# HyperBitGore/deflate.hpp

Measured on AMD Instinct MI355X. Metric: GB/s deflate+inflate on 1 GiB buffer at 1/2/4/8 MI355X; ratio vs reference, higher is better.
Workload: dtype u8; 1 GPU; deflate level 2 + inflate round trip of a per-GPU 1 GiB 'repeat' corpus (SURVEY App. B), device-resident; corpus=repeat, bytes_per_gpu=1073741824, level=2, segment_bytes=32768, parallelism=shard1

## Files before the change

### deflate.hpp_amd/csrc/deflate_kernels.hip

```cpp
#include "dmx_device.h"
#include "dmx_internal.h"
#include "huff_fit.h"

namespace dmx {

constexpr int DF_NT = 1024;
constexpr int DF_CHUNK = 258;
constexpr int df_hash_bits(int seg) {
    return seg >= 32768 ? 12 : 11;
}
constexpr int DF_L3_DEPTH = 16;
constexpr uint32_t DF_L3_LONG = 16;
constexpr uint32_t DF_L3_RP = 512;
constexpr bool df_early(int seg) { return seg >= 32768; }
constexpr uint32_t EM_ALL_LITERALS = 0xFFFFFFFFu;


__device__ __forceinline__ int df_tid() {
    int t = threadIdx.x;
    asm volatile("" : "+v"(t));
    return t;
}

__device__ uint32_t block_excl_scan(uint32_t v, uint32_t* scratch, uint32_t* total) {
// ... 158 lines not shown
    while (L < maxl) {
        const uint32_t o = L + 16 * sub;
        const uint32_t ip = (p + o) >> 2, sp = (p + o) & 3, iq = (q + o) >> 2, sq = (q + o) & 3;
        uint32_t a[5], b[5];
#pragma unroll
        for (int k = 0; k < 5; k++) {
            a[k] = w[ip + k];
            b[k] = w[iq + k];
        }
        uint32_t x = 0, off = 0;
#pragma unroll
        for (int k = 0; k < 4; k++) {
            const uint32_t d = __builtin_amdgcn_alignbyte(a[k + 1], a[k], sp) ^
                               __builtin_amdgcn_alignbyte(b[k + 1], b[k], sq);
            if (!x && d) {
                x = d;
                off = 4 * k;
            }
        }
        uint32_t v = x ? 16 * sub + off + ((uint32_t)__builtin_ctz(x) >> 3) : 64u;
        v = min(v, xor_lane<1>(v));
        v = min(v, xor_lane<2>(v));
        if (v < 64) {
            L += v;
            break;
        }
        L += 64;
    }
    return min(L, maxl);
}

__device__ __forceinline__ uint8_t data_byte(const uint32_t* w, uint32_t p) {
    return (uint8_t)(w[p >> 2] >> ((p & 3) * 8));
}

__device__ __forceinline__ uint32_t fixed_lit_len(uint32_t s) {
    return s < 144 ? 8 : s < 256 ? 9 : s < 280 ? 7 : 8;
}
__device__ __forceinline__ uint32_t fixed_lit_code(uint32_t s) {
    uint32_t c = s < 144 ? 0x30 + s : s < 256 ? 0x190 + (s - 144) : s < 280 ? s - 256 : 0xC0 + (s - 280);
    return bitrev(c, fixed_lit_len(s));
}


template <int SEG, bool EARLY>
struct DfBufs;
template <int SEG>
struct DfBufs<SEG, false> {
    uint32_t data32[SEG / 4 + 32];
    alignas(16) uint16_t cand[SEG + 8];
    alignas(16) uint32_t U[2 << df_hash_bits(SEG)];
};
template <int SEG>
struct DfBufs<SEG, true> {
    static constexpr int BW = SEG / 4 + 32;
    static_assert((2 << df_hash_bits(SEG)) * 4 == SEG, "the table fills an image buffer's SEG bytes");
    alignas(16) uint32_t buf[2][BW];
    alignas(16) uint16_t cand[SEG + 8];
};
template <int SEG>
struct DfSmem : DfBufs<SEG, df_early(SEG)> {
    static constexpr bool EARLY = df_early(SEG);
    static constexpr int NWALK = (SEG + DF_CHUNK - 1) / DF_CHUNK;
    static constexpr int HB = df_hash_bits(SEG);
    static constexpr int HT = 1 << HB;
    static constexpr int UW = 2 * HT;
// ... 122 lines not shown
    uint32_t head = (16u - (off & 15u)) & 15u;
    if (((reinterpret_cast<uintptr_t>(src) + head) & 15) != 0 || head > n) head = n;
    for (uint32_t i = t; i < head; i += DF_NT) dbytes[off + i] = src[i];
    const uint32_t nvec = (n - head) / 16;
    const uint4* s4 = reinterpret_cast<const uint4*>(src + head);
    uint4* d4 = reinterpret_cast<uint4*>(dbytes + off + head);
    for (uint32_t i = t; i < nvec; i += DF_NT) d4[i] = s4[i];
    for (uint32_t i = head + 16 * nvec + t; i < n; i += DF_NT) dbytes[off + i] = src[i];
}

template <int SEG, bool L3, bool BATCH, bool DICT, bool PIPE = false>
__device__ __forceinline__ void deflate_segment(const DeflateArgs& A, DfSmem<SEG>& S, uint64_t seg,
                                                uint32_t& staged, [[maybe_unused]] uint32_t iw) {
    constexpr bool EARLY = DfSmem<SEG>::EARLY;
    uint32_t *data32, *U;
    if constexpr (EARLY) {
        data32 = &S.buf[0][0] + iw;
        U = &S.buf[0][0] + ((uint32_t)DfSmem<SEG>::BW - iw);
    } else {
        data32 = S.data32;
        U = S.U;
    }
    [[maybe_unused]] constexpr int NWALK = DfSmem<SEG>::NWALK;
    constexpr int HT = DfSmem<SEG>::HT;
    constexpr int NMAP = SEG / 32;
    const int t = df_tid();
    const DfSegAddr sa = df_seg_addr<SEG, BATCH, DICT>(A, seg);
    const uint32_t D = DICT ? sa.dlen : 0u;
    const uint32_t nb = D + sa.nb;
    constexpr int level = L3 ? 3 : 2;
    uint8_t* const dbytes = reinterpret_cast<uint8_t*>(data32);
    constexpr bool TERMRUN = !L3 && SEG >= 32768;
    constexpr uint32_t RUN_NONE = 0xFFFFFFFFu;
    DMX_PHASE(A.dbg, seg, 0);

    {
        const uint8_t* src = sa.src;
        const uint32_t nvec = nb / 16;
        if (staged) {
        } else if (DICT && D) {
            df_load_at(dbytes, 0, sa.dict, D, t);
            df_load_at(dbytes, D, src, nb - D, t);
        } else if ((((uintptr_t)src) & 15) == 0) {
            const uint4* s4 = reinterpret_cast<const uint4*>(src);
            uint4* d4 = reinterpret_cast<uint4*>(data32);
            for (uint32_t i = t; i < nvec; i += DF_NT) d4[i] = s4[i];
            for (uint32_t i = nvec * 16 + t; i < nb; i += DF_NT) dbytes[i] = src[i];
        } else {
            for (uint32_t i = t; i < nb; i += DF_NT) dbytes[i] = src[i];
        }
        for (uint32_t i = nb + t; i < ((nb + 3) & ~3u) + 32; i += DF_NT) dbytes[i] = 0;
        if (t < NMAP) S.tokmap[t] = 0;
        if (t == 0) S.sh[46] = 0;
        if (TERMRUN && t == 1) S.sh[45] = RUN_NONE;
        if (TERMRUN && t == 2) S.sh[43] = 0;
        if (t >= 48 && t < 63) S.sh[t] = 0;
        if (level >= 2 && EARLY) {
            uint4* const u4 = reinterpret_cast<uint4*>(U);
            for (int i = t; i < 2 * HT / 4; i += DF_NT) u4[i] = make_uint4(0, 0, 0, 0);
        } else if (level >= 2)
            for (int i = t; i < 2 * HT; i += DF_NT) U[i] = 0;
    }
    if constexpr (EARLY) df_lds_barrier();
    else __syncthreads();
    DMX_PHASE(A.dbg, seg, 1);
    staged = 0;

    if (level != 0) {
        [[maybe_unused]] uint32_t run_lo = RUN_NONE, run_d = 0;
        [[maybe_unused]] uint32_t run_e = RUN_NONE;
        [[maybe_unused]] float run_rcp = 0.f;
        if (level >= 2) {
            constexpr uint32_t HB = DfSmem<SEG>::HB;
            const uint2* const tab = reinterpret_cast<const uint2*>(U);
            uint32_t* const cand32 = reinterpret_cast<uint32_t*>(S.cand);
            constexpr uint32_t NOH = 0xFFFFFFFFu;
            struct RoundState {
                uint32_t h0, h1, p0, f0, f1;
                bool ok0, ok1;
            };
            bool skipped = false;
            auto run_rounds = [&](auto rpc) {
                constexpr uint32_t RP = decltype(rpc)::value;
                constexpr uint32_t NR = SEG / RP;
                constexpr uint32_t TAGB = NR <= 16 ? 4 : NR <= 32 ? 5 : NR <= 64 ? 6 : 7;
                static_assert(NR <= 128, "round number is at most 7 bits");
                constexpr uint32_t FPB = 17 - TAGB;
                const bool act = RP >= 2 * DF_NT || t < (int)(RP / 2);
                const uint32_t tt = RP >= 2 * DF_NT ? (uint32_t)t : (uint32_t)t & (RP / 2 - 1);
                constexpr bool SKIP = RP == 2 * DF_NT;
                uint32_t skip_d = 0, skip_end = 0, wait = 0, backoff = 1;
                skipped = false;
                bool pend = false;
                auto round = [&](uint32_t r0, uint32_t rr, RoundState& cur, const RoundState& prev, auto full) {
                    constexpr bool FULL = decltype(full)::value;
                    const uint32_t p0 = r0 + 2 * tt, p1 = p0 + 1;
                    if (SKIP && skip_d) {
                        if (r0 + RP <= skip_end || (!TERMRUN && skip_end >= nb)) {
                            if (FULL || p0 < nb)
                                cand32[p0 >> 1] = (FULL || p0 + 4 <= nb ? skip_d : 0u) |
                                                  ((FULL || p1 + 4 <= nb ? skip_d : 0u) << 16);
                            cur = RoundState{NOH, NOH, p0, 0, 0, false, false};
                            skipped = true;
                            return;
                        }
                        skip_d = 0;
                    }
                    uint32_t dlr = 0;
                    if (SKIP && pend) dlr = S.sh[44];
                    const uint32_t i0 = p0 >> 2, sh = p0 & 3;
                    const uint32_t wa = data32[i0], wb = data32[i0 + 1];
                    const uint32_t k0 = __builtin_amdgcn_alignbyte(wb, wa, sh);
                    const uint32_t k1 = __builtin_amdgcn_alignbyte(wb, wa, sh + 1);
                    const uint32_t prod0 = k0 * 0x1E35A7BDu;
                    const uint32_t prod1 = k1 * 0x1E35A7BDu;
                    const bool ok0 = act && (FULL || p0 + 4 <= nb), ok1 = act && (FULL || p1 + 4 <= nb);
                    const uint32_t h0 = ok0 ? prod0 >> (32 - HB) : NOH, h1 = ok1 ? prod1 >> (32 - HB) : NOH;
                    const uint32_t fa0 = (prod0 >> (32 - HB - 16)) & 0xFFFFu, fa1 = (prod1 >> (32 - HB - 16)) & 0xFFFFu;
                    const uint32_t hl = (uint32_t)__builtin_amdgcn_update_dpp((int)NOH, (int)h1, 0x111, 0xF, 0xF, false);
                    const uint32_t rtag = rr << (32 - TAGB);
                    if (ok0 && h0 != hl)
                        atomicMax(&U[2 * h0 + 1], rtag | ((0x7FFFu - p0) << FPB) | (fa0 >> (16 - FPB)));
                    if (ok1 && h1 != h0)
                        atomicMax(&U[2 * h1 + 1], rtag | ((0x7FFFu - p1) << FPB) | (fa1 >> (16 - FPB)));
                    const uint32_t hn = (uint32_t)__builtin_amdgcn_update_dpp((int)NOH, (int)(prev.ok0 ? prev.h0 : NOH), 0x101, 0xF, 0xF, false);
                    if (prev.ok0 && prev.h0 != (prev.ok1 ? prev.h1 : NOH))
                        atomicMax(&U[2 * prev.h0], ((prev.p0 + 1) << 16) | prev.f0);
                    if (prev.ok1 && prev.h1 != hn) atomicMax(&U[2 * prev.h1], ((prev.p0 + 2) << 16) | prev.f1);
                    bool tested = false;
                    if (SKIP && pend) {
                        pend = false;
                        uint32_t dl = __builtin_amdgcn_readfirstlane(dlr);
                        wait -= wait ? 1u : 0u;
                        if (!wait && dl) {
                            tested = true;
                            {
                                const uint32_t ki = (uint32_t)t >> 6, k = ki + 2, bq = r0 + 4 * ((uint32_t)t & 63);
                                if (ki < 15 && dl % k == 0 && bq + 4 <= nb) {
                                    const uint32_t dk = dl / k, ia = (bq - dk) >> 2, sk = (bq - dk) & 3;
                                    if (data32[bq >> 2] != __builtin_amdgcn_alignbyte(data32[ia + 1], data32[ia], sk))
                                        atomicMax(&S.sh[48 + ki], rr + 1);
                                }
                            }
                            __syncthreads();
                            uint32_t dsel = dl;
#pragma unroll
                            for (uint32_t k = 2; k <= 16; k++)
                                dsel = (dl % k == 0 && S.sh[48 + k - 2] != rr + 1) ? dl / k : dsel;
                            dl = __builtin_amdgcn_readfirstlane(dsel);
                            skip_d = dl;
                            const uint32_t sa = (r0 - dl) & 3;
                            uint32_t mm = 0xFFFFFFFFu;
#pragma unroll
                            for (int j = 7; j >= 0; j--) {
                                const uint32_t bq = r0 + 4 * ((uint32_t)t + DF_NT * j);
                                if (bq < nb) {
                                    const uint32_t ia = (bq - dl) >> 2;
                                    const uint32_t df = data32[bq >> 2] ^
                                                        __builtin_amdgcn_alignbyte(data32[ia + 1], data32[ia], sa);
                                    mm = df ? bq + ((uint32_t)__builtin_ctz(df) >> 3) : mm;
                                }
                            }
                            if (mm != 0xFFFFFFFFu) atomicMax(&S.sh[46], ((rr + 1) << 16) | (0xFFFFu - mm));
                        }
                    }
                    __syncthreads();
                    if (SKIP && tested) {
                        const uint32_t mt = __builtin_amdgcn_readfirstlane(S.sh[46]);
                        const uint32_t m = (mt >> 16) == rr + 1 ? 0xFFFFu - (mt & 0xFFFFu) : 0xFFFFFFFFu;
                        skip_end = m >= nb ? nb : (m >= 3 ? m - 3 : 0u);
                        if (TERMRUN && skip_end >= nb) {
                            if (t == 0) {
                                S.sh[45] = r0;
                                S.sh[47] = skip_d;
                            }
                            skipped = true;
                            return;
                        }
                        if (r0 + RP <= skip_end || (!TERMRUN && skip_end >= nb)) {
                            if (act && (FULL || p0 < nb))
                                cand32[p0 >> 1] = (ok0 ? skip_d : 0u) | ((ok1 ? skip_d : 0u) << 16);
                            cur = RoundState{NOH, NOH, p0, 0, 0, false, false};
                            backoff = 1;
                            skipped = true;
                            return;
                        }
                        skip_d = 0;
                        wait = backoff;
                        backoff = min(2 * backoff, 16u);
                    }
                    uint2 e0 = tab[ok0 ? h0 : 0u], e1 = tab[ok1 ? h1 : 0u];
                    asm volatile("" : "+v"(e0.x), "+v"(e0.y), "+v"(e1.x), "+v"(e1.y));
                    auto pick = [&](uint2 e, uint32_t p, uint32_t fa, bool ok) -> uint32_t {
                        const uint32_t f = e.y, hd = e.x;
                        const uint32_t q = 0x7FFFu - ((f >> FPB) & 0x7FFFu);
                        const bool fr = ((f >> (32 - TAGB)) == rr) & (q < p) &
                                        ((f & ((1u << FPB) - 1)) == (fa >> (16 - FPB)));
                        const bool lt = (hd != 0u) & ((hd & 0xFFFFu) == fa);
                        const uint32_t c = fr ? p - q : (lt ? p + 1u - (hd >> 16) : 0u);
                        return ok ? c : 0u;
                    };
                    const uint32_t c0 = pick(e0, p0, fa0, ok0), c1 = pick(e1, p1, fa1, ok1);
                    if (act && (FULL || p0 < nb)) cand32[p0 >> 1] = c0 | (c1 << 16);
                    cur = RoundState{h0, h1, p0, fa0, fa1, ok0, ok1};
                    if (SKIP) {
                        if (t >= DF_NT - 64) {
                            const uint32_t nc = (uint32_t)__popcll(__ballot(c0 != 0u)) + (uint32_t)__popcll(__ballot(c1 != 0u));
                            if (t == DF_NT - 1) S.sh[44] = nc >= 120 ? c1 : 0u;
                        }
                        pend = FULL;
                    }
                    __syncthreads();
                };
                using Full = std::integral_constant<bool, true>;
                using Part = std::integral_constant<bool, false>;
                const DeflateArgs& Ar = A;
                RoundState A = {0, 0, 0, 0, 0, false, false}, B = A;
                uint32_t r0 = 0, rr = 0;
                auto more = [&]() { return !(TERMRUN && SKIP) || skip_end < nb; };
                for (; r0 + 2 * RP + 3 <= nb && more(); r0 += 2 * RP, rr += 2) {
                    round(r0, rr, A, B, Full{});
                    if (rr == 0) DMX_PHASE(Ar.dbg, seg, 12);
                    if (!more()) break;
                    round(r0 + RP, rr + 1, B, A, Full{});
                    if (rr == 0) DMX_PHASE(Ar.dbg, seg, 13);
                }
                for (; r0 < nb && more(); r0 += RP, rr++) {
                    round(r0, rr, A, B, Part{});
                    const RoundState x = A;
                    A = B;
                    B = x;
                }
            };
            if (level == 3 && DF_L3_RP != 2 * DF_NT)
                run_rounds(std::integral_constant<uint32_t, DF_L3_RP>{});
            else
                run_rounds(std::integral_constant<uint32_t, 2 * DF_NT>{});
            if (skipped) __syncthreads();
            if (TERMRUN && skipped) {
                run_lo = __builtin_amdgcn_readfirstlane(S.sh[45]);
                run_d = __builtin_amdgcn_readfirstlane(S.sh[47]);
            }
            DMX_PHASE(A.dbg, seg, 14);
        }
        if (level == 3) {
            constexpr int KP = SEG / DF_NT;
            uint32_t best[KP / 2];
#pragma unroll
            for (int k = 0; k < KP; k++) {
                const uint32_t p = t + DF_NT * k;
                uint32_t bd = 0;
                const uint32_t d0 = p < nb && (!DICT || p >= D) ? S.cand[p] : 0u;
                if (d0) {
                    const uint32_t hi = min(D + (p - D) / DF_CHUNK * DF_CHUNK + DF_CHUNK, nb);
                    const uint32_t maxl = min(258u, hi - p);
                    uint32_t q = p - d0;
                    uint32_t bl = matchlen(data32, p, q, min(maxl, DF_L3_LONG));
                    if (bl >= 3) bd = d0;
                    else bl = 2;
                    uint32_t tail = bl >= 3 ? lds_rd32u(data32, p + bl - 3) : 0u;
                    for (int hop = 1; hop < DF_L3_DEPTH && bl < maxl && bl < DF_L3_LONG; hop++) {
                        const uint32_t dq = S.cand[q];
                        if (!dq) break;
                        q -= dq;
                        if (bl >= 3 && lds_rd32u(data32, q + bl - 3) != tail) continue;
                        const uint32_t L = matchlen_u(data32, p, q, maxl);
                        if (L > bl) {
                            bl = L;
                            bd = p - q;
                            tail = lds_rd32u(data32, p + bl - 3);
                        }
                    }
                }
                if (k & 1) best[k / 2] |= bd << 16;
                else best[k / 2] = bd;
            }
            __syncthreads();
#pragma unroll
            for (int k = 0; k < KP; k++) {
                const uint32_t p = t + DF_NT * k;
                if (p < nb) S.cand[p] = (uint16_t)(k & 1 ? best[k / 2] >> 16 : best[k / 2] & 0xFFFFu);
            }
            __syncthreads();
        }
        if (level >= 2) {
            for (uint32_t w = t; w < NMAP; w += DF_NT) {
                if (TERMRUN && 32 * w >= run_lo) {
                    const uint32_t b0 = 32 * w;
                    S.mmap[w] = nb >= b0 + 35 ? 0xFFFFFFFFu : (nb > b0 + 3 ? (1u << (nb - 3 - b0)) - 1u : 0u);
                    continue;
                }
                const uint4* c4 = reinterpret_cast<const uint4*>(S.cand + 32 * w);
                uint32_t m = 0;
#pragma unroll
                for (int k = 0; k < 4; k++) {
                    const uint4 v = c4[k];
                    const uint32_t x[4] = {v.x, v.y, v.z, v.w};
#pragma unroll
                    for (int j = 0; j < 4; j++) {
                        m |= ((x[j] & 0xFFFFu) ? 1u : 0u) << (8 * k + 2 * j);
                        m |= ((x[j] >> 16) ? 1u : 0u) << (8 * k + 2 * j + 1);
                    }
                }
                const uint32_t b0 = 32 * w;
                S.mmap[w] = b0 + 32 <= nb ? m : (nb > b0 ? m & ((1u << (nb - b0)) - 1u) : 0u);
            }
            if (TERMRUN && run_lo != RUN_NONE) {
                const uint32_t v = run_d | (run_d << 16);
                const uint32_t i0 = run_lo / 8, i1 = max(i0, (nb - 11) / 8 + 1);
                uint4* const c4 = reinterpret_cast<uint4*>(S.cand);
                for (uint32_t i = i0 + t; i < i1; i += DF_NT) c4[i] = make_uint4(v, v, v, v);
                const uint32_t p = 8 * i1 + t;
                if (t < 16 && p < nb) S.cand[p] = (uint16_t)(p + 4 <= nb ? run_d : 0u);
                constexpr uint32_t RP = 2 * DF_NT;
                const uint32_t bq = run_lo - RP + 4 * (uint32_t)t;
                if ((uint32_t)t < RP / 4 && bq >= run_d) {
                    const uint32_t ia = (bq - run_d) >> 2;
                    const uint32_t df = data32[bq >> 2] ^
                                        __builtin_amdgcn_alignbyte(data32[ia + 1], data32[ia], (run_lo - run_d) & 3);
                    if (df) atomicMax(&S.sh[43], ((run_lo / RP + 1) << 16) | (bq + 4 - ((uint32_t)__builtin_clz(df) >> 3)));
                }
            }
            __syncthreads();
            if (TERMRUN && run_lo != RUN_NONE) {
                constexpr uint32_t RP = 2 * DF_NT;
                const uint32_t et = __builtin_amdgcn_readfirstlane(S.sh[43]);
                run_e = (et >> 16) == run_lo / RP + 1 ? et & 0xFFFFu : max(run_lo - RP, (run_d + 3) & ~3u);
                run_rcp = __builtin_amdgcn_rcpf((float)run_d);
            }
        }
        DMX_PHASE(A.dbg, seg, 2);
        if constexpr (EARLY) staged = df_prefetch_next<SEG, BATCH, DICT, PIPE>(A, seg, U);

        constexpr uint32_t CH = DF_CHUNK;
        const uint32_t nwalk = (nb - D + CH - 1) / CH;
        auto parse_walk = [&](auto runc) {
            constexpr bool RUNW = decltype(runc)::value;
            const uint32_t sub = t & 3;
            const bool lead = sub == 0;
            const uint32_t lo = D + (t >> 2) * CH;
            const uint32_t hi = min(lo + CH, nb);
            auto bits_range = [](uint32_t a, uint32_t b, uint32_t w) -> uint32_t {
                const uint32_t e = b - w * 32;
                return (e >= 32 ? 0xFFFFFFFFu : ((1u << e) - 1u)) & (0xFFFFFFFFu << (a & 31));
            };
            [[maybe_unused]] auto known_len = [&](uint32_t q, uint32_t d) -> bool {
                const uint32_t m = (uint32_t)((float)d * run_rcp + 0.5f);
                return (q >= run_e) & (m * run_d == d) & (q - d + run_d >= run_e);
            };
            auto len_at = [&](uint32_t q, uint32_t d, uint32_t maxl) -> uint32_t {
                if (!RUNW) return matchlen4(data32, q, q - d, maxl, sub);
                const bool kn = known_len(q, d);
                const uint32_t L = matchlen4(data32, q, q - d, kn ? 0u : maxl, sub);
                return kn ? maxl : L;
            };
            auto full_len = [&](uint32_t q) -> uint32_t {
                return len_at(q, S.cand[q], min(258u, hi - q));
            };
            uint32_t p = lo, w = lo >> 5, mw = S.mmap[w], tok = 0, lastp = lo;
            auto mbit = [&](uint32_t q) -> bool {
                return (S.mmap[q >> 5] >> (q & 31)) & 1u;
            };
            while (p < hi) {
                const uint32_t wi = p >> 5;
                if (wi != w) {
                    if (tok && lead) atomicOr(&S.tokmap[w], tok);
                    w = wi;
                    mw = S.mmap[w];
                    tok = 0;
                }
                const uint32_t m = mw & (0xFFFFFFFFu << (p & 31));
                const uint32_t q = m ? w * 32 + __builtin_ctz(m) : 0xFFFFFFFFu;
                if (q >= hi || !m) {
                    uint32_t e = min((w + 1) * 32, hi);
                    tok |= bits_range(p, e, w);
                    if (RUNW && e < hi) {
                        const uint32_t wl = w + 1 + sub, b0 = wl * 32;
                        const bool in = b0 < hi;
                        uint32_t x = in ? S.mmap[wl] : 0u;
                        x = in && hi - b0 < 32 ? x & ((1u << (hi - b0)) - 1u) : x;
                        uint32_t f = (!in || x) ? sub : 4u;
                        f = min(f, xor_lane<1>(f));
                        f = min(f, xor_lane<2>(f));
                        if (sub < f) atomicOr(&S.tokmap[wl], bits_range(b0, min(b0 + 32, hi), wl));
                        e = min((w + 1 + f) * 32, hi);
                    }
                    lastp = e - 1;
                    p = e;
                    continue;
                }
                tok |= bits_range(p, q, w);
                p = q;
// ... 124 lines not shown
                                atomicOr(&S.tokmap[e >> 5], 1u << (e & 31));
                                if (r == 2) atomicOr(&S.tokmap[(e + 1) >> 5], 1u << ((e + 1) & 31));
                            }
                            S.cand[s0 + 1] = (uint16_t)Lx;
                            if (r >= 3) {
                                S.cand[e] = (uint16_t)dq;
                                S.cand[e + 1] = (uint16_t)r;
                            } else if (r) {
                                S.cand[e] = 0;
                                if (r == 2) S.cand[e + 1] = 0;
                            }
                            for (uint32_t wi = s0 >> 5; wi <= (sync - 1) >> 5; wi++) {
                                const uint32_t a = max(s0, wi * 32) - wi * 32, z = min(sync, wi * 32 + 32) - wi * 32;
                                const uint32_t rm = (z >= 32 ? 0xFFFFFFFFu : ((1u << z) - 1u)) & (0xFFFFFFFFu << a);
                                nb0 = (s0 >> 5) == wi ? 1u << (s0 & 31) : 0u;
                                nb1 = (r && (e >> 5) == wi ? 1u << (e & 31) : 0u) |
                                      (r == 2 && ((e + 1) >> 5) == wi ? 1u << ((e + 1) & 31) : 0u);
                                atomicAnd(&S.tokmap[wi], ~rm | nb0 | nb1);
                            }
                        }
                    }
                }
            }
            __syncthreads();
        }

        bool by_word = false;
        if constexpr (TERMRUN) {
            static_assert(NMAP == DF_NT, "one token-start bitmap word per thread");
            by_word = run_lo != RUN_NONE;
        }
        if (by_word) {
            const uint32_t m = S.tokmap[t];
            const uint4* const c4 = reinterpret_cast<const uint4*>(S.cand + 32 * t);
            uint32_t nz = 0;
#pragma unroll
            for (int k = 0; k < 4; k++) {
                const uint4 v = c4[k];
                const uint32_t x[4] = {v.x, v.y, v.z, v.w};
#pragma unroll
                for (int j = 0; j < 4; j++) {
                    nz |= ((x[j] & 0xFFFFu) ? 1u : 0u) << (8 * k + 2 * j);
                    nz |= ((x[j] >> 16) ? 1u : 0u) << (8 * k + 2 * j + 1);
                }
            }
            const uint32_t mt = m & nz, lt = m & ~nz;
            const uint32_t chain = lt & (lt << 1) & (lt << 2) & (lt << 3);
            uint32_t ws = lt & ~(lt << 1);
#pragma unroll
            for (int i = 0; i < 10; i++) ws |= (ws << 3) & chain;
            const uint32_t val = ((uint32_t)__popc(m) << 16) | ((uint32_t)__popc(mt) + (uint32_t)__popc(ws));
            const uint32_t inc = wave_incl_scan(val);
            uint32_t* const sc = S.scan + DF_NT / 64;
            if ((t & 63) == 63) sc[t >> 6] = inc;
            __syncthreads();
            uint32_t ex = inc - val, tot = 0;
#pragma unroll
            for (int i = 0; i < DF_NT / 64; i++) {
                const uint32_t x = sc[i];
                if (i < (t >> 6)) ex += x;
                tot += x;
            }
            DMX_PHASE(A.dbg, seg, 15);
            if ((tot >> 16) == nb - D) {
                if (t == 0) A.ntok[seg] = EM_ALL_LITERALS;
            } else {
                uint32_t* dst = A.tok + seg * (uint64_t)A.tok_stride + (ex & 0xFFFFu);
                const uint32_t* const sw = reinterpret_cast<const uint32_t*>(&S);
                const uint32_t cbase = (uint32_t)(reinterpret_cast<const uint32_t*>(S.cand) - sw) + 16 * (uint32_t)t;
                const uint32_t dbase = (uint32_t)(data32 - sw) + 8 * (uint32_t)t;
                uint32_t all = mt | ws;
                while (all) {
                    uint32_t b[4], lo[4], hi[4];
                    bool on[4];
#pragma unroll
                    for (int i = 0; i < 4; i++) {
                        on[i] = all != 0;
                        b[i] = on[i] ? (uint32_t)__builtin_ctz(all) : 0u;
                        all &= all - 1;
                        const uint32_t at = (mt >> b[i]) & 1u ? cbase + (b[i] >> 1) : dbase + (b[i] >> 2);
                        lo[i] = sw[at];
                        hi[i] = sw[at + 1];
                    }
#pragma unroll
                    for (int i = 0; i < 4; i++) {
                        if (on[i]) {
                            const bool mat = (mt >> b[i]) & 1u;
                            const uint32_t v = __builtin_amdgcn_alignbyte(hi[i], lo[i], mat ? 2 * (b[i] & 1) : b[i] & 3);
                            const uint32_t x = lt >> b[i], c = 1 + ((x >> 1) & 1u) + ((x >> 1) & (x >> 2) & 1u);
                            *dst++ = mat ? 0x80000000u | (((v >> 16) - 3) << 16) | ((v & 0xFFFFu) - 1)
                                         : (v & (0xFFFFFFu >> (24 - 8 * c))) | (c << 24);
                        }
                    }
                }
                if (t == 0) A.ntok[seg] = tot & 0xFFFFu;
            }
        } else {
            TokRange tr;
            uint32_t tr_total;
            {
                const uint32_t c = t < NMAP ? (uint32_t)__popc(S.tokmap[t]) : 0u;
                uint32_t tot;
                const uint32_t ex = block_excl_scan(c, S.scan, &tot);
                if (t < NMAP) S.mmap[t] = ex;
                __syncthreads();
                tr_total = tot;
                const uint32_t K = (tot + DF_NT - 1) / DF_NT;
                const uint32_t first = min((uint32_t)t * K, tot);
                tr.n = min(first + K, tot) - first;
                uint32_t lo = 0, hi = NMAP;
                while (hi - lo > 1) {
                    const uint32_t mid = (lo + hi) >> 1;
                    if (S.mmap[mid] <= first) lo = mid;
                    else hi = mid;
                }
                tr.w = lo;
                const uint32_t m = S.tokmap[lo];
                uint32_t b = 0, k = tr.n ? first - S.mmap[lo] : 0u;
    #pragma unroll
                for (uint32_t sh = 16; sh >= 1; sh >>= 1) {
                    const uint32_t c = (uint32_t)__popc((m >> b) & ((1u << sh) - 1u));
                    const bool up = k >= c;
                    b += up ? sh : 0u;
                    k -= up ? c : 0u;
                }
                tr.m = m & (0xFFFFFFFFu << b);
            }
            DMX_PHASE(A.dbg, seg, 15);
// ... 319 lines not shown
    uint32_t mis;
    uint32_t nb;
    uint32_t ntok;
    bool raw;
    __device__ uint32_t raw_word(uint32_t k) const {
        const uint32_t x = 4 * k + mis;
        const uint32_t a = inw[x >> 2];
        const uint32_t b = (x >> 2) + 1 < in_words_end ? inw[(x >> 2) + 1] : 0u;
        return mis ? __builtin_amdgcn_alignbyte(b, a, x & 3) : a;
    }
    __device__ void load4(uint32_t blk, uint32_t (&v)[4]) const {
        const uint32_t i0 = blk * 256 + 4 * lane_id();
#pragma unroll
        for (int j = 0; j < 4; j++) v[j] = 0;
        if (raw) {
#pragma unroll
            for (int j = 0; j < 4; j++)
                if (i0 + j < ntok) v[j] = raw_word(i0 + j);
        } else if (i0 + 3 < ntok) {
            const uint4 q = *reinterpret_cast<const uint4*>(tok + i0);
            v[0] = q.x, v[1] = q.y, v[2] = q.z, v[3] = q.w;
        } else {
#pragma unroll
            for (int j = 0; j < 4; j++)
                if (i0 + j < ntok) v[j] = tok[i0 + j];
        }
    }
    __device__ uint32_t count_of(uint32_t v, uint32_t idx) const {
        if (raw) return min(4u, nb - 4 * idx);
        return (v >> 31) ? 0u : (v >> 24) & 3u;
    }
};
template <bool RAW>
__device__ EmSrc em_src(const DeflateArgs& A, uint64_t fseg, const uint8_t* inb, uint64_t tail, uint32_t nb) {
    EmSrc s;
    s.mis = (uint32_t)(reinterpret_cast<uintptr_t>(inb) & 3);
    s.inw = reinterpret_cast<const uint32_t*>(inb - s.mis);
    s.in_words_end = (tail + s.mis + 3) / 4;
    s.nb = nb;
    s.raw = RAW || A.ntok[fseg] == EM_ALL_LITERALS;
    s.ntok = s.raw ? (nb + 3) / 4 : A.ntok[fseg];
    s.tok = s.raw ? nullptr : A.tok + fseg * (uint64_t)A.tok_stride;
    return s;
}

__device__ __forceinline__ uint32_t em_stored_hdr(uint32_t q, bool fin, uint32_t len) {
    return q == 0 ? (fin ? 1u : 0u) : q == 1 ? len & 0xFFu : q == 2 ? (len >> 8) & 0xFFu
         : q == 3 ? ~len & 0xFFu : (~len >> 8) & 0xFFu;
}

template <int SEG, bool RAW, bool BATCH>
__device__ void em_segment(const DeflateArgs& A, EmWave& W, uint64_t seg_of_wave) {
    static_assert(!BATCH || SEG <= 32768, "a batch does not pair front segments into 64 KiB blocks");
    const uint64_t seg = (uint64_t)(uint32_t)__builtin_amdgcn_readfirstlane((int)(uint32_t)seg_of_wave) |
                         ((uint64_t)(uint32_t)__builtin_amdgcn_readfirstlane((int)(uint32_t)(seg_of_wave >> 32)) << 32);
    constexpr uint32_t NH = SEG > 32768 ? 2u : 1u;
    constexpr uint32_t HB = (uint32_t)SEG / NH;
    const int lane = lane_id();
    EM_PHASE(A.dbg, seg, 4);
    const DfSegAddr sa = df_seg_addr<SEG, BATCH>(A, seg);
    const uint32_t nb = sa.nb;
    const uint32_t np = (nb + HB - 1) / HB;
    const bool is_final = sa.is_last && A.final_last;
    uint32_t* const slot = reinterpret_cast<uint32_t*>(A.slots + seg * (uint64_t)A.slot_bytes);
    auto part = [&](uint32_t h) {
        return em_src<RAW>(A, seg * NH + h, sa.src + (uint64_t)h * HB, sa.tail - (uint64_t)h * HB, min(HB, nb - h * HB));
    };
    const uint32_t nsto = nb > 65535u ? 2u : 1u;
    const uint32_t n1 = nsto == 2 ? 32768u : nb;
    const uint64_t stored_bytes = 5ull * nsto + nb + (is_final ? 0 : 5);

    if (A.level != 0) {
        const EmSrc S0 = part(0);
        uint32_t v0[4] = {0, 0, 0, 0};
        if (S0.ntok) S0.load4(0, v0);
        for (int i = lane; i < EM_SYM; i += 64) W.freq[i] = 0;
        wave_sync();
        for (uint32_t h = 0; h < np; h++) {
            const EmSrc S = h == 0 ? S0 : part(h);
            const uint32_t nblk = (S.ntok + 255) / 256;
            for (uint32_t blk = 0; blk < nblk; blk++) {
                uint32_t v[4];
                if (h == 0 && blk == 0) {
#pragma unroll
                    for (int j = 0; j < 4; j++) v[j] = v0[j];
                } else {
                    S.load4(blk, v);
                }
#pragma unroll
                for (int j = 0; j < 4; j++) {
                    const uint32_t idx = blk * 256 + 4 * lane + j;
                    if (idx >= S.ntok) continue;
                    if (!S.raw && (v[j] >> 31)) {
                        atomicAdd(&W.freq[len_sym(((v[j] >> 16) & 0xFFu) + 3)], 1u);
                        atomicAdd(&W.freq[EM_LIT + dist_sym((v[j] & 0x7FFFu) + 1)], 1u);
                    } else {
                        const uint32_t cnt = S.count_of(v[j], idx);
#pragma unroll
                        for (uint32_t i = 0; i < 4u; i++)
                            if (i < cnt) atomicAdd(&W.freq[(v[j] >> (8 * i)) & 0xFFu], 1u);
                    }
                }
            }
        }
        wave_sync();
        if (lane == 0) atomicAdd(&W.freq[256], 1u);
        wave_sync();
        EM_PHASE(A.dbg, seg, 5);
        const EmCodes ec = em_build_codes(W);
        EM_PHASE(A.dbg, seg, 6);
        const uint32_t nlit = ec.nlit, ndist = ec.ndist, nall = nlit + ndist;
        auto seqv = [&](uint32_t i) -> uint32_t { return i < nlit ? W.len[i] : W.len[EM_LIT + i - nlit]; };
        uint64_t rm[5];
        if (lane < 20) W.prefreq[lane] = 0;
#pragma unroll
        for (int c = 0; c < 5; c++) {
            const uint32_t i = 64 * c + lane;
            bool start = false;
// ... 71 lines not shown
                if (use_dyn) h |= ((uint64_t)(nlit - 257) << 3) | ((uint64_t)(ndist - 1) << 8) | ((uint64_t)(hclen - 4) << 13);
                em_put(W.stg, 0, h, use_dyn ? 17 : 3);
            }
            if (use_dyn) {
                if (lane < (int)hclen) em_put(W.stg, 17 + 3 * lane, pv, 3);
                const uint32_t rb = 17 + 3 * hclen;
#pragma unroll
                for (int c = 0; c < 5; c++) {
                    const uint32_t rl = run[c] & 511u;
                    if (!rl) continue;
                    const uint32_t v = (run[c] >> 9) & 15u;
                    const RunPlan p = plan_run(v, rl);
                    uint32_t pos = rb + (run[c] >> 13);
                    auto put = [&](uint32_t sym, uint32_t extra, uint32_t xb) {
                        const uint32_t pc = W.precode[sym];
                        const uint32_t l = pc >> 16;
                        em_put(W.stg, pos, (uint64_t)(pc & 0xFFFFu) | ((uint64_t)extra << l), l + xb);
                        pos += l + xb;
                    };
                    if (v == 0) {
                        for (uint32_t q = 0; q < p.n18; q++) put(18, (q + 1 == p.n18 ? p.last18 : 138) - 11, 7);
                        if (p.n17) put(17, p.r17 - 3, 3);
                        for (uint32_t q = 0; q < p.nlit; q++) put(0, 0, 0);
                    } else {
                        put(v, 0, 0);
                        for (uint32_t q = 0; q < p.n16; q++) put(16, (q + 1 == p.n16 ? p.last16 : 6) - 3, 2);
                        for (uint32_t q = 1; q < p.nlit; q++) put(v, 0, 0);
                    }
                }
            }
            wave_sync();
            uint32_t cur = 3 + (use_dyn ? hdr_bits : 0u);
            uint32_t* dst = slot;
            for (uint32_t h = 0; h < np; h++) {
                const EmSrc S = h == 0 ? S0 : part(h);
                const uint32_t nblk = (S.ntok + 255) / 256;
                for (uint32_t blk = 0; blk < nblk; blk++) {
                    uint32_t v[4], nbit[4];
                    uint64_t pat[4];
                    if (h == 0 && blk == 0) {
#pragma unroll
                        for (int j = 0; j < 4; j++) v[j] = v0[j];
                    } else {
                        S.load4(blk, v);
                    }
                    uint32_t mine = 0;
#pragma unroll
                    for (int j = 0; j < 4; j++) {
                        const uint32_t idx = blk * 256 + 4 * lane + j;
                        nbit[j] = 0;
                        pat[j] = 0;
                        if (idx < S.ntok) pat[j] = em_pattern(W, v[j], S.count_of(v[j], idx), nbit[j], S.raw);
                        mine += nbit[j];
                    }
                    const uint32_t inc = wave_incl_scan(mine);
                    uint32_t pos = cur + inc - mine;
#pragma unroll
                    for (int j = 0; j < 4; j++) {
                        em_put(W.stg, pos, pat[j], nbit[j]);
                        pos += nbit[j];
                    }
                    cur += __shfl(inc, 63, 64);
                    wave_sync();
                    if (cur >= 32u * EM_FLUSH) {
                        const uint32_t nw = cur >> 5;
                        em_flush(W.stg, dst, nw);
                        dst += nw;
                        cur &= 31;
                    }
                }
            }
            EM_PHASE(A.dbg, seg, 8);
            const uint32_t eob = W.code[256];
            if (lane == 0) em_put(W.stg, cur, eob & 0xFFFFu, eob >> 16);
            const uint32_t end_bits = cur + (eob >> 16);
// ... 420 lines not shown
```

Measured before the change: 481.3 GB/s.

## Encode leading literal prefix as raw span and compact non-zero mask via dot2

In the run-terminated path, the kernel finds the first match position per segment and packs the literal prefix before it into a raw-literal span. That span's length is recorded in the upper bits of ntok, so fewer literal tokens are written. The emitter now walks each part as two sources, a raw prefix followed by the token stream. Separately, the per-thread non-zero candidate mask is computed with packed min and udot2 instructions instead of many compare and shift steps. This adds an atomicMin, a ballot and a more complex offset computation, and changes the ntok encoding consumed by the emitter.

```diff
diff --git a/deflate.hpp_amd/csrc/deflate_kernels.hip b/deflate.hpp_amd/csrc/deflate_kernels.hip
--- a/deflate.hpp_amd/csrc/deflate_kernels.hip
+++ b/deflate.hpp_amd/csrc/deflate_kernels.hip
@@ -214,6 +214,25 @@
 
 __device__ __forceinline__ uint8_t data_byte(const uint32_t* w, uint32_t p) {
     return (uint8_t)(w[p >> 2] >> ((p & 3) * 8));
+}
+
+typedef unsigned short df_u16x2 __attribute__((ext_vector_type(2)));
+__device__ __forceinline__ uint32_t df_nonzero32(const uint4* c4) {
+    uint32_t acc[2] = {0, 0};
+#pragma unroll
+    for (int k = 0; k < 4; k++) {
+        const uint4 v = c4[k];
+        const uint32_t x[4] = {v.x, v.y, v.z, v.w};
+#pragma unroll
+        for (int j = 0; j < 4; j++) {
+            const int e = (4 * k + j) & 7;
+            const df_u16x2 w = {(unsigned short)(1u << (2 * e)), (unsigned short)(2u << (2 * e))};
+            uint32_t f;
+            asm("v_pk_min_u16 %0, %1, %2" : "=v"(f) : "v"(x[j]), "s"(0x00010001u));
+            acc[k >> 1] = __builtin_amdgcn_udot2(__builtin_bit_cast(df_u16x2, f), w, acc[k >> 1], false);
+        }
+    }
+    return acc[0] | (acc[1] << 16);
 }
 
 __device__ __forceinline__ uint32_t fixed_lit_len(uint32_t s) {
@@ -682,6 +701,7 @@
                 for (uint32_t i = i0 + t; i < i1; i += DF_NT) c4[i] = make_uint4(v, v, v, v);
                 const uint32_t p = 8 * i1 + t;
                 if (t < 16 && p < nb) S.cand[p] = (uint16_t)(p + 4 <= nb ? run_d : 0u);
+                if (t == 16) S.sh[42] = RUN_NONE;
                 constexpr uint32_t RP = 2 * DF_NT;
                 const uint32_t bq = run_lo - RP + 4 * (uint32_t)t;
                 if ((uint32_t)t < RP / 4 && bq >= run_d) {
@@ -918,18 +938,7 @@
         }
         if (by_word) {
             const uint32_t m = S.tokmap[t];
-            const uint4* const c4 = reinterpret_cast<const uint4*>(S.cand + 32 * t);
-            uint32_t nz = 0;
-#pragma unroll
-            for (int k = 0; k < 4; k++) {
-                const uint4 v = c4[k];
-                const uint32_t x[4] = {v.x, v.y, v.z, v.w};
-#pragma unroll
-                for (int j = 0; j < 4; j++) {
-                    nz |= ((x[j] & 0xFFFFu) ? 1u : 0u) << (8 * k + 2 * j);
-                    nz |= ((x[j] >> 16) ? 1u : 0u) << (8 * k + 2 * j + 1);
-                }
-            }
+            const uint32_t nz = df_nonzero32(reinterpret_cast<const uint4*>(S.cand + 32 * t));
             const uint32_t mt = m & nz, lt = m & ~nz;
             const uint32_t chain = lt & (lt << 1) & (lt << 2) & (lt << 3);
             uint32_t ws = lt & ~(lt << 1);
@@ -939,7 +948,10 @@
             const uint32_t inc = wave_incl_scan(val);
             uint32_t* const sc = S.scan + DF_NT / 64;
             if ((t & 63) == 63) sc[t >> 6] = inc;
+            if (const uint64_t hm = __ballot(mt != 0); mt != 0 && (uint32_t)__builtin_ctzll(hm) == ((uint32_t)t & 63u))
+                atomicMin(&S.sh[42], 32 * (uint32_t)t + (uint32_t)__builtin_ctz(mt));
             __syncthreads();
+            const uint32_t first = S.sh[42];
             uint32_t ex = inc - val, tot = 0;
 #pragma unroll
             for (int i = 0; i < DF_NT / 64; i++) {
@@ -951,7 +963,25 @@
             if ((tot >> 16) == nb - D) {
                 if (t == 0) A.ntok[seg] = EM_ALL_LITERALS;
             } else {
-                uint32_t* dst = A.tok + seg * (uint64_t)A.tok_stride + (ex & 0xFFFFu);
+                const uint32_t P1 = __builtin_amdgcn_readfirstlane(first);
+                const uint32_t C = D + ((P1 - D) & ~3u);
+                uint32_t K = 0, woff = ex & 0xFFFFu;
+                if (C != D) {
+                    const auto c3 = [](uint32_t k) -> uint32_t { return (k * 43 + 86) >> 7; };
+                    const uint32_t w0 = D >> 5, w1 = P1 >> 5;
+                    const uint32_t was = w0 == w1 ? c3(P1 - D) : c3(32 - (D & 31)) + 11 * (w1 - w0 - 1) + c3(P1 & 31);
+                    const uint32_t now = C < P1 ? 1u + ((C >> 5) != w1 && (P1 & 31) ? 1u : 0u) : 0u;
+                    K = was - now;
+                    const uint32_t B = 32 * (uint32_t)t;
+                    woff -= K;
+                    if (B < P1) {
+                        const uint32_t lo = max(B, C), hi = min(B + 32, P1);
+                        ws &= P1 - B >= 32 ? 0u : 0xFFFFFFFFu << (P1 - B);
+                        if (lo < hi) ws |= 1u << (lo - B);
+                        woff = B > C ? 1u : 0u;
+                    }
+                }
+                uint32_t* dst = A.tok + seg * (uint64_t)A.tok_stride + woff;
                 const uint32_t* const sw = reinterpret_cast<const uint32_t*>(&S);
                 const uint32_t cbase = (uint32_t)(reinterpret_cast<const uint32_t*>(S.cand) - sw) + 16 * (uint32_t)t;
                 const uint32_t dbase = (uint32_t)(data32 - sw) + 8 * (uint32_t)t;
@@ -979,7 +1009,7 @@
                         }
                     }
                 }
-                if (t == 0) A.ntok[seg] = tot & 0xFFFFu;
+                if (t == 0) A.ntok[seg] = ((tot & 0xFFFFu) - K) | ((C - D) << 14);
             }
         } else {
             TokRange tr;
@@ -1365,15 +1395,23 @@
     }
 };
 template <bool RAW>
-__device__ EmSrc em_src(const DeflateArgs& A, uint64_t fseg, const uint8_t* inb, uint64_t tail, uint32_t nb) {
+__device__ EmSrc em_src(const DeflateArgs& A, uint64_t fseg, const uint8_t* inb, uint64_t tail, uint32_t nb, uint32_t k) {
     EmSrc s;
     s.mis = (uint32_t)(reinterpret_cast<uintptr_t>(inb) & 3);
     s.inw = reinterpret_cast<const uint32_t*>(inb - s.mis);
     s.in_words_end = (tail + s.mis + 3) / 4;
-    s.nb = nb;
-    s.raw = RAW || A.ntok[fseg] == EM_ALL_LITERALS;
-    s.ntok = s.raw ? (nb + 3) / 4 : A.ntok[fseg];
-    s.tok = s.raw ? nullptr : A.tok + fseg * (uint64_t)A.tok_stride;
+    const uint32_t nt = RAW ? EM_ALL_LITERALS : A.ntok[fseg];
+    const bool all = nt == EM_ALL_LITERALS;
+    s.raw = k == 0;
+    if (k == 0) {
+        s.nb = all ? nb : (nt >> 16) * 4;
+        s.ntok = (s.nb + 3) / 4;
+        s.tok = nullptr;
+    } else {
+        s.nb = nb;
+        s.ntok = all ? 0u : nt & 0xFFFFu;
+        s.tok = A.tok + fseg * (uint64_t)A.tok_stride;
+    }
     return s;
 }
 
@@ -1396,27 +1434,30 @@
     const uint32_t np = (nb + HB - 1) / HB;
     const bool is_final = sa.is_last && A.final_last;
     uint32_t* const slot = reinterpret_cast<uint32_t*>(A.slots + seg * (uint64_t)A.slot_bytes);
-    auto part = [&](uint32_t h) {
-        return em_src<RAW>(A, seg * NH + h, sa.src + (uint64_t)h * HB, sa.tail - (uint64_t)h * HB, min(HB, nb - h * HB));
+    constexpr uint32_t NK = RAW ? 1u : 2u;
+    auto part = [&](uint32_t h, uint32_t k) {
+        return em_src<RAW>(A, seg * NH + h, sa.src + (uint64_t)h * HB, sa.tail - (uint64_t)h * HB, min(HB, nb - h * HB), k);
     };
     const uint32_t nsto = nb > 65535u ? 2u : 1u;
     const uint32_t n1 = nsto == 2 ? 32768u : nb;
     const uint64_t stored_bytes = 5ull * nsto + nb + (is_final ? 0 : 5);
 
     if (A.level != 0) {
-        const EmSrc S0 = part(0);
-        uint32_t v0[4] = {0, 0, 0, 0};
+        const EmSrc S0 = part(0, 0), S1 = part(0, NK - 1);
+        uint32_t v0[4] = {0, 0, 0, 0}, v1[4] = {0, 0, 0, 0};
         if (S0.ntok) S0.load4(0, v0);
+        if (NK > 1 && S1.ntok) S1.load4(0, v1);
         for (int i = lane; i < EM_SYM; i += 64) W.freq[i] = 0;
         wave_sync();
-        for (uint32_t h = 0; h < np; h++) {
-            const EmSrc S = h == 0 ? S0 : part(h);
+        for (uint32_t hk = 0; hk < NK * np; hk++) {
+            const uint32_t h = hk / NK, k = hk % NK;
+            const EmSrc S = h ? part(h, k) : k ? S1 : S0;
             const uint32_t nblk = (S.ntok + 255) / 256;
             for (uint32_t blk = 0; blk < nblk; blk++) {
                 uint32_t v[4];
                 if (h == 0 && blk == 0) {
 #pragma unroll
-                    for (int j = 0; j < 4; j++) v[j] = v0[j];
+                    for (int j = 0; j < 4; j++) v[j] = k ? v1[j] : v0[j];
                 } else {
                     S.load4(blk, v);
                 }
@@ -1554,15 +1595,16 @@
             wave_sync();
             uint32_t cur = 3 + (use_dyn ? hdr_bits : 0u);
             uint32_t* dst = slot;
-            for (uint32_t h = 0; h < np; h++) {
-                const EmSrc S = h == 0 ? S0 : part(h);
+            for (uint32_t hk = 0; hk < NK * np; hk++) {
+                const uint32_t h = hk / NK, k = hk % NK;
+                const EmSrc S = h ? part(h, k) : k ? S1 : S0;
                 const uint32_t nblk = (S.ntok + 255) / 256;
                 for (uint32_t blk = 0; blk < nblk; blk++) {
                     uint32_t v[4], nbit[4];
                     uint64_t pat[4];
                     if (h == 0 && blk == 0) {
 #pragma unroll
-                        for (int j = 0; j < 4; j++) v[j] = v0[j];
+                        for (int j = 0; j < 4; j++) v[j] = k ? v1[j] : v0[j];
                     } else {
                         S.load4(blk, v);
                     }
```

Measured after the change: 481.0 GB/s. No clear change (-0.1%).

## Test pending run before hashing and precompute literal prefix before first match

Applied to the files above, without the earlier changes.

The pending periodic-run test in the hash-insertion rounds is moved ahead of the hash and atomic work, so a round confirmed to lie inside a repeat run skips its own hashing and table updates. The code also records the first match-candidate position after the dictionary. It marks every byte before that position as a literal in the token map, and parse walkers start at that position instead of scanning the literal prefix. This is aimed at the highly repetitive corpus and removes redundant hash rounds and parse iterations. In exchange it adds an extra barrier in the test path and more state bookkeeping in shared slots 46 and 47.

```diff
diff --git a/deflate.hpp_amd/csrc/deflate_kernels.hip b/deflate.hpp_amd/csrc/deflate_kernels.hip
--- a/deflate.hpp_amd/csrc/deflate_kernels.hip
+++ b/deflate.hpp_amd/csrc/deflate_kernels.hip
@@ -402,6 +402,7 @@
     uint8_t* const dbytes = reinterpret_cast<uint8_t*>(data32);
     constexpr bool TERMRUN = !L3 && SEG >= 32768;
     constexpr uint32_t RUN_NONE = 0xFFFFFFFFu;
+    constexpr bool LITPREFIX = TERMRUN;
     DMX_PHASE(A.dbg, seg, 0);
 
     {
@@ -440,6 +441,7 @@
         [[maybe_unused]] uint32_t run_lo = RUN_NONE, run_d = 0;
         [[maybe_unused]] uint32_t run_e = RUN_NONE;
         [[maybe_unused]] float run_rcp = 0.f;
+        [[maybe_unused]] uint32_t run_fm = 0;
         if (level >= 2) {
             constexpr uint32_t HB = DfSmem<SEG>::HB;
             const uint2* const tab = reinterpret_cast<const uint2*>(U);
@@ -480,6 +482,76 @@
                     if (SKIP && pend) dlr = S.sh[44];
                     const uint32_t i0 = p0 >> 2, sh = p0 & 3;
                     const uint32_t wa = data32[i0], wb = data32[i0 + 1];
+                    auto run_test = [&](uint32_t dl) {
+                        {
+                            const uint32_t ki = (uint32_t)t >> 6, k = ki + 2, bq = r0 + 4 * ((uint32_t)t & 63);
+                            if (ki < 15 && dl % k == 0 && bq + 4 <= nb) {
+                                const uint32_t dk = dl / k, ia = (bq - dk) >> 2, sk = (bq - dk) & 3;
+                                if (data32[bq >> 2] != __builtin_amdgcn_alignbyte(data32[ia + 1], data32[ia], sk))
+                                    atomicMax(&S.sh[48 + ki], rr + 1);
+                            }
+                        }
+                        __syncthreads();
+                        uint32_t dsel = dl;
+#pragma unroll
+                        for (uint32_t k = 2; k <= 16; k++)
+                            dsel = (dl % k == 0 && S.sh[48 + k - 2] != rr + 1) ? dl / k : dsel;
+                        dl = __builtin_amdgcn_readfirstlane(dsel);
+                        skip_d = dl;
+                        const uint32_t sa = (r0 - dl) & 3;
+                        uint32_t mm = 0xFFFFFFFFu;
+#pragma unroll
+                        for (int j = 7; j >= 0; j--) {
+                            const uint32_t bq = r0 + 4 * ((uint32_t)t + DF_NT * j);
+                            if (bq < nb) {
+                                const uint32_t ia = (bq - dl) >> 2;
+                                const uint32_t df = data32[bq >> 2] ^
+                                                    __builtin_amdgcn_alignbyte(data32[ia + 1], data32[ia], sa);
+                                mm = df ? bq + ((uint32_t)__builtin_ctz(df) >> 3) : mm;
+                            }
+                        }
+                        if (mm != 0xFFFFFFFFu) atomicMax(&S.sh[46], ((rr + 1) << 16) | (0xFFFFu - mm));
+                    };
+                    auto tested_end = [&]() -> uint32_t {
+                        const uint32_t mt = __builtin_amdgcn_readfirstlane(S.sh[46]);
+                        const uint32_t m = (mt >> 16) == rr + 1 ? 0xFFFFu - (mt & 0xFFFFu) : 0xFFFFFFFFu;
+                        return m >= nb ? nb : (m >= 3 ? m - 3 : 0u);
+                    };
+                    constexpr bool TESTFIRST = TERMRUN && SKIP;
+                    if (TESTFIRST && pend) {
+                        pend = false;
+                        const uint32_t dl = __builtin_amdgcn_readfirstlane(dlr);
+                        wait -= wait ? 1u : 0u;
+                        if (!wait && dl) {
+                            run_test(dl);
+                            __syncthreads();
+                            skip_end = tested_end();
+                            if (skip_end >= nb) {
+                                if (t == 0) {
+                                    S.sh[45] = r0;
+                                    S.sh[47] = skip_d | (LITPREFIX ? 0xFFFF0000u : 0u);
+                                }
+                                skipped = true;
+                                return;
+                            }
+                            if (r0 + RP <= skip_end) {
+                                const uint32_t hn = (uint32_t)__builtin_amdgcn_update_dpp((int)NOH, (int)(prev.ok0 ? prev.h0 : NOH), 0x101, 0xF, 0xF, false);
+                                if (prev.ok0 && prev.h0 != (prev.ok1 ? prev.h1 : NOH))
+                                    atomicMax(&U[2 * prev.h0], ((prev.p0 + 1) << 16) | prev.f0);
+                                if (prev.ok1 && prev.h1 != hn) atomicMax(&U[2 * prev.h1], ((prev.p0 + 2) << 16) | prev.f1);
+                                if (FULL || p0 < nb)
+                                    cand32[p0 >> 1] = (FULL || p0 + 4 <= nb ? skip_d : 0u) |
+                                                      ((FULL || p1 + 4 <= nb ? skip_d : 0u) << 16);
+                                cur = RoundState{NOH, NOH, p0, 0, 0, false, false};
+                                backoff = 1;
+                                skipped = true;
+                                return;
+                            }
+                            skip_d = 0;
+                            wait = backoff;
+                            backoff = min(2 * backoff, 16u);
+                        }
+                    }
                     const uint32_t k0 = __builtin_amdgcn_alignbyte(wb, wa, sh);
                     const uint32_t k1 = __builtin_amdgcn_alignbyte(wb, wa, sh + 1);
                     const uint32_t prod0 = k0 * 0x1E35A7BDu;
@@ -498,56 +570,19 @@
                         atomicMax(&U[2 * prev.h0], ((prev.p0 + 1) << 16) | prev.f0);
                     if (prev.ok1 && prev.h1 != hn) atomicMax(&U[2 * prev.h1], ((prev.p0 + 2) << 16) | prev.f1);
                     bool tested = false;
-                    if (SKIP && pend) {
+                    if (!TESTFIRST && SKIP && pend) {
                         pend = false;
-                        uint32_t dl = __builtin_amdgcn_readfirstlane(dlr);
+                        const uint32_t dl = __builtin_amdgcn_readfirstlane(dlr);
                         wait -= wait ? 1u : 0u;
                         if (!wait && dl) {
                             tested = true;
-                            {
-                                const uint32_t ki = (uint32_t)t >> 6, k = ki + 2, bq = r0 + 4 * ((uint32_t)t & 63);
-                                if (ki < 15 && dl % k == 0 && bq + 4 <= nb) {
-                                    const uint32_t dk = dl / k, ia = (bq - dk) >> 2, sk = (bq - dk) & 3;
-                                    if (data32[bq >> 2] != __builtin_amdgcn_alignbyte(data32[ia + 1], data32[ia], sk))
-                                        atomicMax(&S.sh[48 + ki], rr + 1);
-                                }
-                            }
-                            __syncthreads();
-                            uint32_t dsel = dl;
-#pragma unroll
-                            for (uint32_t k = 2; k <= 16; k++)
-                                dsel = (dl % k == 0 && S.sh[48 + k - 2] != rr + 1) ? dl / k : dsel;
-                            dl = __builtin_amdgcn_readfirstlane(dsel);
-                            skip_d = dl;
-                            const uint32_t sa = (r0 - dl) & 3;
-                            uint32_t mm = 0xFFFFFFFFu;
-#pragma unroll
-                            for (int j = 7; j >= 0; j--) {
-                                const uint32_t bq = r0 + 4 * ((uint32_t)t + DF_NT * j);
-                                if (bq < nb) {
-                                    const uint32_t ia = (bq - dl) >> 2;
-                                    const uint32_t df = data32[bq >> 2] ^
-                                                        __builtin_amdgcn_alignbyte(data32[ia + 1], data32[ia], sa);
-                                    mm = df ? bq + ((uint32_t)__builtin_ctz(df) >> 3) : mm;
-                                }
-                            }
-                            if (mm != 0xFFFFFFFFu) atomicMax(&S.sh[46], ((rr + 1) << 16) | (0xFFFFu - mm));
+                            run_test(dl);
                         }
                     }
                     __syncthreads();
-                    if (SKIP && tested) {
-                        const uint32_t mt = __builtin_amdgcn_readfirstlane(S.sh[46]);
-                        const uint32_t m = (mt >> 16) == rr + 1 ? 0xFFFFu - (mt & 0xFFFFu) : 0xFFFFFFFFu;
-                        skip_end = m >= nb ? nb : (m >= 3 ? m - 3 : 0u);
-                        if (TERMRUN && skip_end >= nb) {
-                            if (t == 0) {
-                                S.sh[45] = r0;
-                                S.sh[47] = skip_d;
-                            }
-                            skipped = true;
-                            return;
-                        }
-                        if (r0 + RP <= skip_end || (!TERMRUN && skip_end >= nb)) {
+                    if (!TESTFIRST && SKIP && tested) {
+                        skip_end = tested_end();
+                        if (r0 + RP <= skip_end || skip_end >= nb) {
                             if (act && (FULL || p0 < nb))
                                 cand32[p0 >> 1] = (ok0 ? skip_d : 0u) | ((ok1 ? skip_d : 0u) << 16);
                             cur = RoundState{NOH, NOH, p0, 0, 0, false, false};
@@ -609,7 +644,8 @@
             if (skipped) __syncthreads();
             if (TERMRUN && skipped) {
                 run_lo = __builtin_amdgcn_readfirstlane(S.sh[45]);
-                run_d = __builtin_amdgcn_readfirstlane(S.sh[47]);
+                run_d = __builtin_amdgcn_readfirstlane(S.sh[47]) & 0xFFFFu;
+                if (LITPREFIX) asm volatile("" : "+s"(run_d));
             }
             DMX_PHASE(A.dbg, seg, 14);
         }
@@ -654,10 +690,16 @@
             __syncthreads();
         }
         if (level >= 2) {
+            [[maybe_unused]] uint32_t mfirst = RUN_NONE;
             for (uint32_t w = t; w < NMAP; w += DF_NT) {
                 if (TERMRUN && 32 * w >= run_lo) {
                     const uint32_t b0 = 32 * w;
-                    S.mmap[w] = nb >= b0 + 35 ? 0xFFFFFFFFu : (nb > b0 + 3 ? (1u << (nb - 3 - b0)) - 1u : 0u);
+                    const uint32_t v = nb >= b0 + 35 ? 0xFFFFFFFFu : (nb > b0 + 3 ? (1u << (nb - 3 - b0)) - 1u : 0u);
+                    S.mmap[w] = v;
+                    if (LITPREFIX) {
+                        const uint32_t x = b0 + 32 <= D ? 0u : (b0 < D ? v & (0xFFFFFFFFu << (D & 31)) : v);
+                        mfirst = x ? b0 + (uint32_t)__builtin_ctz(x) : RUN_NONE;
+                    }
                     continue;
                 }
                 const uint4* c4 = reinterpret_cast<const uint4*>(S.cand + 32 * w);
@@ -673,7 +715,17 @@
                     }
                 }
                 const uint32_t b0 = 32 * w;
-                S.mmap[w] = b0 + 32 <= nb ? m : (nb > b0 ? m & ((1u << (nb - b0)) - 1u) : 0u);
+                const uint32_t v = b0 + 32 <= nb ? m : (nb > b0 ? m & ((1u << (nb - b0)) - 1u) : 0u);
+                S.mmap[w] = v;
+                if (LITPREFIX) {
+                    const uint32_t x = b0 + 32 <= D ? 0u : (b0 < D ? v & (0xFFFFFFFFu << (D & 31)) : v);
+                    mfirst = x ? b0 + (uint32_t)__builtin_ctz(x) : RUN_NONE;
+                }
+            }
+            if (LITPREFIX && run_lo != RUN_NONE) {
+                const uint64_t has = __ballot(mfirst != RUN_NONE);
+                if (has && ((uint32_t)t & 63u) == (uint32_t)__builtin_ctzll(has))
+                    atomicMin(&S.sh[47], (mfirst << 16) | run_d);
             }
             if (TERMRUN && run_lo != RUN_NONE) {
                 const uint32_t v = run_d | (run_d << 16);
@@ -695,8 +747,16 @@
             if (TERMRUN && run_lo != RUN_NONE) {
                 constexpr uint32_t RP = 2 * DF_NT;
                 const uint32_t et = __builtin_amdgcn_readfirstlane(S.sh[43]);
+                [[maybe_unused]] const uint32_t fw = LITPREFIX ? (uint32_t)__builtin_amdgcn_readfirstlane(S.sh[47]) : 0u;
                 run_e = (et >> 16) == run_lo / RP + 1 ? et & 0xFFFFu : max(run_lo - RP, (run_d + 3) & ~3u);
                 run_rcp = __builtin_amdgcn_rcpf((float)run_d);
+                if (LITPREFIX) {
+                    run_fm = min(fw >> 16, nb);
+                    const uint32_t a = max(D, 32u * (uint32_t)t), b = min(run_fm, 32u * (uint32_t)t + 32u);
+                    if (a < b)
+                        atomicOr(&S.tokmap[t], (b - 32u * (uint32_t)t >= 32 ? 0xFFFFFFFFu : ((1u << (b & 31)) - 1u)) &
+                                                   (0xFFFFFFFFu << (a & 31)));
+                }
             }
         }
         DMX_PHASE(A.dbg, seg, 2);
@@ -727,7 +787,10 @@
             auto full_len = [&](uint32_t q) -> uint32_t {
                 return len_at(q, S.cand[q], min(258u, hi - q));
             };
-            uint32_t p = lo, w = lo >> 5, mw = S.mmap[w], tok = 0, lastp = lo;
+            uint32_t p = lo;
+            if (RUNW && LITPREFIX) p = min(max(lo, run_fm), hi);
+            uint32_t lastp = RUNW && LITPREFIX ? min(p, hi - 1) : lo;
+            uint32_t w = lastp >> 5, mw = S.mmap[w], tok = 0;
             auto mbit = [&](uint32_t q) -> bool {
                 return (S.mmap[q >> 5] >> (q & 31)) & 1u;
             };
```

After: 475.0 GB/s before, 506.8 GB/s after (median of 6 runs). 1.07x the previous value.
